# UoL-SignalProcessingGroup/SMC-NUTS

Hardware: AMD Instinct MI355X
Metric: leapfrog-steps/sec (higher is better)
Workload: dtype f64

## Files before the change

include/smcnuts_hip.h:

```cpp
#ifndef SMCNUTS_HIP_H
#define SMCNUTS_HIP_H

#include <stddef.h>
#include <stdint.h>

#ifdef __cplusplus
extern "C" {
#endif

typedef struct smcn_ctx smcn_ctx;

#define SMCN_MODEL_GAUSS 0
#define SMCN_MODEL_ARMA 1
#define SMCN_MODEL_PRMWCD 2
#define SMCN_MODEL_HOST 3
#define SMCN_MODEL_GLM 4
#define SMCN_MODEL_HGLM 5
#define SMCN_MODEL_CATEGORICAL 6
#define SMCN_MODEL_ORDINAL 7
#define SMCN_MODEL_MLGLM 8
#define SMCN_MODEL_WGLM 9
#define SMCN_MODEL_OGLM 10

#define SMCN_LKERNEL_FORWARD 0
// ... 46 lines not shown
int smcn_set_nuts_cap(smcn_ctx* ctx, int doublings, int widen);
int smcn_nuts_parked(smcn_ctx* ctx, int64_t* parked);
int smcn_set_nuts_requeue(smcn_ctx* ctx, int doublings);

int smcn_propose_nuts(smcn_ctx* ctx, double step_size, double phi, int max_depth, double delta_max,
                      int64_t iteration, const double* tape, const int64_t* tape_off);
int smcn_get_tree_stats(smcn_ctx* ctx, int32_t* nleap, int32_t* depth, int32_t* ndraws, int32_t* flags);
int smcn_last_leapfrogs(smcn_ctx* ctx, int64_t* total);
int smcn_get_density_parts(smcn_ctx* ctx, double* lpri0, double* llik0, double* lpri1, double* llik1);

int smcn_reweight(smcn_ctx* ctx, int lkernel);
int smcn_accept_reject(smcn_ctx* ctx, double phi, const double* u, int64_t iteration);
int smcn_reweight_asymptotic(smcn_ctx* ctx, double phi_old, double phi_new);
int smcn_set_logw_density_ratio(smcn_ctx* ctx, double phi_num, double phi_den);

int smcn_set_lkernel_values(smcn_ctx* ctx, const double* L, const double* q);

int smcn_gauss_lkernel_sums(smcn_ctx* ctx, const double* shift, double* sums);
int smcn_gauss_lkernel_logpdf(smcn_ctx* ctx, const double* mu_x, const double* m0, const double* B,
                              const double* U, double c0);
int smcn_gauss_lkernel_device(smcn_ctx* ctx, double info[4]);
int smcn_gauss_lkernel_buffers(smcn_ctx* ctx, int world, void** local_dev, void** gathered_dev);
int smcn_gauss_lkernel_stage(smcn_ctx* ctx, int stage, int world, double n_total, double info[4] );

int smcn_temper_partials(smcn_ctx* ctx, double phi_old, double phi_new, double out[4]);
int smcn_temper_bisect(smcn_ctx* ctx, double phi_old, double target, double* phi, int* status);
int smcn_temper_bisect_pass(smcn_ctx* ctx, int pass, double phi_old);
int smcn_temper_bisect_buffers(smcn_ctx* ctx, int world, void** local, void** gathered);
int smcn_temper_bisect_decide(smcn_ctx* ctx, int pass, int world, double target, double phi_old);
int smcn_temper_bisect_result(smcn_ctx* ctx, double* phi, int* status);

int smcn_eval_proposed_parts(smcn_ctx* ctx, int which);

int smcn_commit(smcn_ctx* ctx, int64_t* n_moved);

int smcn_fast_begin(smcn_ctx* ctx, int64_t K, int save_history, int world);
int smcn_fast_buffers(smcn_ctx* ctx, void** local_partials, void** gathered, int* nq);
int smcn_set_resample_uniforms(smcn_ctx* ctx, const double* u);
int smcn_step_begin(smcn_ctx* ctx, int64_t k);
int smcn_step_finish(smcn_ctx* ctx, int64_t k, int world, int rank, double n_total, double step_size,
                     double phi, int max_depth, double delta_max, int lkernel, int last,
                     const double* tape, const int64_t* tape_off);
int smcn_fast_read(smcn_ctx* ctx, double* hist, double* x_saved, double* logw_saved);
int smcn_fast_read_from(smcn_ctx* ctx, double* hist, double* x_saved, double* logw_saved, int64_t k_from);
int smcn_history_download(smcn_ctx* ctx, int64_t k_from, int64_t k_to, double* x_saved, double* logw_saved);
int smcn_fuse_begin(smcn_ctx* ctx, int Bmax, int world);
int smcn_fuse_buffers(smcn_ctx* ctx, void** local_partials, void** gathered, int* nq);
int smcn_fuse_run(smcn_ctx* ctx, int64_t k0, int B, int world, int rank, double n_total, double step_size,
                  double phi, int max_depth, double delta_max, int decided);
int smcn_fuse_decide(smcn_ctx* ctx, int64_t k0, int world, int rank, double n_total, double phi, int* resample);

typedef int (*smcn_host_target_fn)(void* user, int64_t n, int D, const double* x, int want_grad, double* lpri,
                                   double* llik, double* gpri, double* glik);
int smcn_set_host_target(smcn_ctx* ctx, smcn_host_target_fn fn, void* user);
int smcn_moment_sums_of(smcn_ctx* ctx, const double* v, int Dc, const double* shift, double* out);

int smcn_block_resample_local(smcn_ctx* ctx, int64_t k0);
int smcn_block_launch(smcn_ctx* ctx, int64_t k0, int B, double step_size, double phi, int max_depth,
                      double delta_max);
int smcn_block_post(smcn_ctx* ctx, int64_t k0, int B, int world);
int smcn_block_partials_get(smcn_ctx* ctx, int B, double* out);
int smcn_block_partials_set(smcn_ctx* ctx, int B, int world, const double* gathered);
int smcn_block_stats(smcn_ctx* ctx, int64_t k0, int B, int world, int rank, double n_total, double phi,
                     int final_block );
int smcn_block_wait(smcn_ctx* ctx, int B, int* n_ok, int* resample_next);
int smcn_block_commit(smcn_ctx* ctx, int64_t k0, int n_ok);
int smcn_block_ess(smcn_ctx* ctx, int B, double* out);
int smcn_fuse_finish(smcn_ctx* ctx, int64_t k0, int B, int world, int rank, double n_total, double phi,
                     int* n_ok);
#ifdef SMCN_LEGACY_ABI
int smcn_fuse_partials_get(smcn_ctx* ctx, int B, double* out);
int smcn_fuse_partials_set(smcn_ctx* ctx, int B, int world, const double* in);
#endif

int smcn_partials_get(smcn_ctx* ctx, double* out);
int smcn_partials_set_gathered(smcn_ctx* ctx, const double* in, int world);

int smcn_timers(smcn_ctx* ctx, double out[6], int reset);

int smcn_selftest_math(smcn_ctx* ctx, const double* x, int64_t n, double* out);
int smcn_measure_peaks(smcn_ctx* ctx, double out[3]);
int smcn_device_cache_trim(int device, int64_t* released_bytes, int64_t* idle_bytes);
int smcn_selftest_wide(smcn_ctx* ctx, int lanes, const double* x, int64_t n, double* out);

int smcn_comm_unique_id(char out[128]);
int smcn_comm_init(smcn_ctx* ctx, int rank, int world, const char id[128]);
int smcn_comm_destroy(smcn_ctx* ctx);
int smcn_comm_info(smcn_ctx* ctx, int out[3]);
int smcn_comm_allgather(smcn_ctx* ctx, const void* src_dev, void* dst_dev, int64_t n_doubles);
int smcn_comm_allgather_host(smcn_ctx* ctx, const double* src, int64_t n_doubles, double* dst );
int smcn_comm_alltoallv(smcn_ctx* ctx, const void* send_dev, const int64_t* send_counts, void* recv_dev,
                        const int64_t* recv_counts, int elem_doubles);
int smcn_buf_get(smcn_ctx* ctx, const void* dev, int64_t n_doubles, double* host);
int smcn_buf_set(smcn_ctx* ctx, void* dev, int64_t n_doubles, const double* host);
int smcn_buf_copy(smcn_ctx* ctx, void* dst_dev, const void* src_dev, int64_t n_doubles);

int smcn_gres_begin(smcn_ctx* ctx, int world, double* ttot_host );
int smcn_gres_buffers(smcn_ctx* ctx, void** ttot_local, void** ttot_all, void** keys_send, void** keys_recv,
                      void** rows_send, void** rows_recv);
int smcn_gres_plan(smcn_ctx* ctx, int world, int rank, const double* ttot_all_host ,
                   int64_t iteration, int32_t* dest_rank_host );
int smcn_gres_set_order(smcn_ctx* ctx, const int32_t* order );
int smcn_gres_reserve(smcn_ctx* ctx, int64_t n_requests_to_serve);
int smcn_gres_serve(smcn_ctx* ctx, int world, int rank, int64_t n_requests);
int smcn_gres_finish(smcn_ctx* ctx, int world, const double* loglik );

int smcn_bench_resample(smcn_ctx* ctx, int reps, int64_t iteration, double* ms_total);

int smcn_pointwise_dims(const smcn_ctx* ctx, int64_t* n_obs, int* n_cols);
int smcn_pointwise_loglik(smcn_ctx* ctx, const double* x , int64_t M, double* out );
int smcn_pointwise_partials(smcn_ctx* ctx, const double* x_or_null , const double* logw_or_null ,
                            int64_t M, double* out );
int smcn_pointwise_last_ms(const smcn_ctx* ctx, double* ms);

int smcn_psis_candidates(smcn_ctx* ctx, const double* x_or_null , const double* logw_or_null ,
                         int64_t M, double mw, int64_t S, double* cand );
int smcn_psis_body(smcn_ctx* ctx, const double* x_or_null , const double* logw_or_null , int64_t M,
                   double mw, int64_t S, const double* cutoff , double* body );
int smcn_psis_fit(smcn_ctx* ctx, const double* cand , const double* body ,
                  int64_t n_obs, double mw, int64_t S, double* out );
int smcn_psis_loo(smcn_ctx* ctx, const double* x_or_null , const double* logw_or_null , int64_t M,
                  double* out , double* head_or_null );
int smcn_psis_last_ms(const smcn_ctx* ctx, double* ms );

int smcn_predict_set_data(smcn_ctx* ctx, const double* block, int64_t len, int has_y);
int smcn_predict_dims(smcn_ctx* ctx, int64_t* n_rows, int* n_cols, int* has_y);
int smcn_predict_loglik(smcn_ctx* ctx, const double* x , int64_t M, double* out );
int smcn_predict_partials(smcn_ctx* ctx, const double* x_or_null , const double* logw_or_null ,
                          int64_t M, double* out );
int smcn_predict_last_ms(const smcn_ctx* ctx, double* ms);

int smcn_predict_draws(smcn_ctx* ctx, const double* x_or_null , const double* logw_or_null , int64_t M,
                       int64_t S, uint64_t seed, const int64_t* ancestors_or_null ,
                       const int64_t* new_group_or_null , int64_t s_first, int64_t s_count,
                       double* y_out , int64_t* ancestors_out , int64_t* n_bad_out);
int smcn_predict_draws_last_ms(const smcn_ctx* ctx, double* ms);

int smcn_summary_begin(smcn_ctx* ctx, const double* x_or_null , const double* logw_or_null ,
                       const double* v_or_null , int64_t M, int Dv, double* head_out );
int smcn_summary_weights(smcn_ctx* ctx, double lw_max, double lw_sum, double* mass_out);
int smcn_summary_select(smcn_ctx* ctx, int nq, const double* thresholds );
int smcn_summary_hist(smcn_ctx* ctx, int pass, int nq, double* out );
int smcn_summary_descend(smcn_ctx* ctx, int pass, int nq, const int32_t* digits ,
                         const double* residual );
int smcn_summary_values(smcn_ctx* ctx, int nq, double* out , double* nan_flags_out );
int smcn_summary_cdf(smcn_ctx* ctx, int T, const double* at , double* out );
int smcn_summary_last_ms(const smcn_ctx* ctx, double* ms);
int smcn_summary_pass_ms(const smcn_ctx* ctx, double* ms );

int smcn_cov_partials(smcn_ctx* ctx, double lw_max, const double* centre_or_null , int64_t slices,
                      double* out , double* centre_out );
int smcn_cov_dims(const smcn_ctx* ctx, int64_t* out );
int smcn_cov_last_ms(const smcn_ctx* ctx, double* ms);

int smcn_debug_profile(smcn_ctx* ctx, uint64_t out[16], int reset);

#ifdef __cplusplus
}
#endif
#endif
```

smcnuts_amd/_capi.py:

```python
import ctypes as C
import os

import numpy as np

from . import build as _build

MODEL_GAUSS, MODEL_ARMA, MODEL_PRMWCD, MODEL_HOST = 0, 1, 2, 3
MODEL_GLM = 4
MODEL_HGLM = 5
MODEL_CATEGORICAL = 6
MODEL_ORDINAL = 7
MODEL_MLGLM = 8
MODEL_WGLM = 9
MODEL_OGLM = 10
HOST_TARGET_FN = C.CFUNCTYPE(C.c_int, C.c_void_p, C.c_int64, C.c_int, C.POINTER(C.c_double), C.c_int,
                             C.POINTER(C.c_double), C.POINTER(C.c_double), C.POINTER(C.c_double),
                             C.POINTER(C.c_double))
LKERNEL_FORWARD, LKERNEL_GAUSSIAN = 0, 1

_dp = C.POINTER(C.c_double)
_ip = C.POINTER(C.c_int32)
_lp = C.POINTER(C.c_int64)
_ctx = C.c_void_p

# ... 4 lines not shown
    "smcn_ctx_destroy": ([_ctx], None),
    "smcn_dim": ([_ctx], C.c_int),
    "smcn_constrained_dim": ([_ctx], C.c_int),
    "smcn_fused_transitions": ([_ctx], C.c_int),
    "smcn_set_stream": ([_ctx, C.c_void_p], C.c_int),
    "smcn_synchronize": ([_ctx], C.c_int),
    "smcn_set_seed": ([_ctx, C.c_uint64], C.c_int),
    "smcn_set_state": ([_ctx, _dp, _dp], C.c_int),
    "smcn_get_state": ([_ctx, _dp, _dp, _dp], C.c_int),
    "smcn_get_proposal": ([_ctx, _dp, _dp, _dp, _dp], C.c_int),
    "smcn_set_momentum": ([_ctx, _dp], C.c_int),
    "smcn_set_proposal": ([_ctx, _dp, _dp, _dp], C.c_int),
    "smcn_target_eval": ([_ctx, _dp, C.c_int64, C.c_double, _dp, _dp, _dp, _dp], C.c_int),
    "smcn_target_constrain": ([_ctx, _dp, C.c_int64, _dp], C.c_int),
    "smcn_init_particles_std_normal": ([_ctx, C.c_double], C.c_int),
    "smcn_init_weights": ([_ctx, C.c_double, _dp], C.c_int),
    "smcn_normalise_partials": ([_ctx, _dp], C.c_int),
    "smcn_normalise_apply": ([_ctx, C.c_double], C.c_int),
    "smcn_normalise": ([_ctx, _dp, _dp], C.c_int),
    "smcn_moment_sums": ([_ctx, _dp, _dp], C.c_int),
    "smcn_resample_multinomial": ([_ctx, _dp, C.c_double, C.c_double, C.c_int64, _lp], C.c_int),
    "smcn_propose_nuts": ([_ctx, C.c_double, C.c_double, C.c_int, C.c_double, C.c_int64, _dp, _lp], C.c_int),
    "smcn_get_tree_stats": ([_ctx, _ip, _ip, _ip, _ip], C.c_int),
    "smcn_last_leapfrogs": ([_ctx, _lp], C.c_int),
    "smcn_get_density_parts": ([_ctx, _dp, _dp, _dp, _dp], C.c_int),
    "smcn_set_lkernel_values": ([_ctx, _dp, _dp], C.c_int),
    "smcn_reweight": ([_ctx, C.c_int], C.c_int),
    "smcn_accept_reject": ([_ctx, C.c_double, _dp, C.c_int64], C.c_int),
    "smcn_reweight_asymptotic": ([_ctx, C.c_double, C.c_double], C.c_int),
    "smcn_set_logw_density_ratio": ([_ctx, C.c_double, C.c_double], C.c_int),
    "smcn_gauss_lkernel_sums": ([_ctx, _dp, _dp], C.c_int),
    "smcn_gauss_lkernel_logpdf": ([_ctx, _dp, _dp, _dp, _dp, C.c_double], C.c_int),
    "smcn_gauss_lkernel_device": ([_ctx, _dp], C.c_int),
    "smcn_gauss_lkernel_buffers": ([_ctx, C.c_int, C.POINTER(C.c_void_p), C.POINTER(C.c_void_p)], C.c_int),
    "smcn_gauss_lkernel_stage": ([_ctx, C.c_int, C.c_int, C.c_double, _dp], C.c_int),
    "smcn_set_nuts_cap": ([_ctx, C.c_int, C.c_int], C.c_int),
    "smcn_set_nuts_requeue": ([_ctx, C.c_int], C.c_int),
    "smcn_nuts_parked": ([_ctx, C.POINTER(C.c_int64)], C.c_int),
    "smcn_temper_partials": ([_ctx, C.c_double, C.c_double, _dp], C.c_int),
    "smcn_temper_bisect": ([_ctx, C.c_double, C.c_double, C.POINTER(C.c_double), C.POINTER(C.c_int)], C.c_int),
    "smcn_temper_bisect_pass": ([_ctx, C.c_int, C.c_double], C.c_int),
    "smcn_temper_bisect_buffers": ([_ctx, C.c_int, C.POINTER(C.c_void_p), C.POINTER(C.c_void_p)], C.c_int),
    "smcn_temper_bisect_decide": ([_ctx, C.c_int, C.c_int, C.c_double, C.c_double], C.c_int),
    "smcn_temper_bisect_result": ([_ctx, C.POINTER(C.c_double), C.POINTER(C.c_int)], C.c_int),
    "smcn_eval_proposed_parts": ([_ctx, C.c_int], C.c_int),
    "smcn_commit": ([_ctx, _lp], C.c_int),
    "smcn_fast_begin": ([_ctx, C.c_int64, C.c_int, C.c_int], C.c_int),
    "smcn_fast_buffers": ([_ctx, C.POINTER(C.c_void_p), C.POINTER(C.c_void_p), C.POINTER(C.c_int)], C.c_int),
    "smcn_set_resample_uniforms": ([_ctx, _dp], C.c_int),
    "smcn_step_begin": ([_ctx, C.c_int64], C.c_int),
    "smcn_step_finish": ([_ctx, C.c_int64, C.c_int, C.c_int, C.c_double, C.c_double, C.c_double, C.c_int,
                          C.c_double, C.c_int, C.c_int, _dp, _lp], C.c_int),
    "smcn_fast_read": ([_ctx, _dp, _dp, _dp], C.c_int),
    "smcn_fast_read_from": ([_ctx, _dp, _dp, _dp, C.c_int64], C.c_int),
    "smcn_history_download": ([_ctx, C.c_int64, C.c_int64, _dp, _dp], C.c_int),
    "smcn_fuse_begin": ([_ctx, C.c_int, C.c_int], C.c_int),
    "smcn_fuse_buffers": ([_ctx, C.POINTER(C.c_void_p), C.POINTER(C.c_void_p), C.POINTER(C.c_int)], C.c_int),
    "smcn_fuse_run": ([_ctx, C.c_int64, C.c_int, C.c_int, C.c_int, C.c_double, C.c_double, C.c_double, C.c_int,
                       C.c_double, C.c_int], C.c_int),
    "smcn_set_resample_scheme": ([_ctx, C.c_int], C.c_int),
    "smcn_set_wide_eval": ([_ctx, C.c_int], C.c_int),
    "smcn_set_lane_grid": ([_ctx, C.c_int64], C.c_int),
    "smcn_set_lane_segments": ([_ctx, C.c_int], C.c_int),
    "smcn_set_host_target": ([_ctx, HOST_TARGET_FN, C.c_void_p], C.c_int),
    "smcn_moment_sums_of": ([_ctx, _dp, C.c_int, _dp, _dp], C.c_int),
    "smcn_block_resample_local": ([_ctx, C.c_int64], C.c_int),
    "smcn_block_launch": ([_ctx, C.c_int64, C.c_int, C.c_double, C.c_double, C.c_int, C.c_double], C.c_int),
    "smcn_block_post": ([_ctx, C.c_int64, C.c_int, C.c_int], C.c_int),
    "smcn_block_partials_get": ([_ctx, C.c_int, _dp], C.c_int),
    "smcn_block_partials_set": ([_ctx, C.c_int, C.c_int, _dp], C.c_int),
    "smcn_block_stats": ([_ctx, C.c_int64, C.c_int, C.c_int, C.c_int, C.c_double, C.c_double, C.c_int], C.c_int),
    "smcn_block_wait": ([_ctx, C.c_int, C.POINTER(C.c_int), C.POINTER(C.c_int)], C.c_int),
    "smcn_block_commit": ([_ctx, C.c_int64, C.c_int], C.c_int),
    "smcn_block_ess": ([_ctx, C.c_int, _dp], C.c_int),
    "smcn_fuse_decide": ([_ctx, C.c_int64, C.c_int, C.c_int, C.c_double, C.c_double, C.POINTER(C.c_int)], C.c_int),
    "smcn_fuse_finish": ([_ctx, C.c_int64, C.c_int, C.c_int, C.c_int, C.c_double, C.c_double,
                          C.POINTER(C.c_int)], C.c_int),
    "smcn_partials_get": ([_ctx, _dp], C.c_int),
    "smcn_partials_set_gathered": ([_ctx, _dp, C.c_int], C.c_int),
    "smcn_timers": ([_ctx, _dp, C.c_int], C.c_int),
    "smcn_selftest_math": ([_ctx, _dp, C.c_int64, _dp], C.c_int),
    "smcn_measure_peaks": ([_ctx, _dp], C.c_int),
    "smcn_selftest_wide": ([_ctx, C.c_int, _dp, C.c_int64, _dp], C.c_int),
    "smcn_device_cache_trim": ([C.c_int, C.POINTER(C.c_int64), C.POINTER(C.c_int64)], C.c_int),
    "smcn_debug_profile": ([_ctx, C.POINTER(C.c_uint64), C.c_int], C.c_int),
    "smcn_bench_resample": ([_ctx, C.c_int, C.c_int64, _dp], C.c_int),
    "smcn_comm_unique_id": ([C.c_char_p], C.c_int),
    "smcn_comm_init": ([_ctx, C.c_int, C.c_int, C.c_char_p], C.c_int),
    "smcn_comm_destroy": ([_ctx], C.c_int),
    "smcn_comm_info": ([_ctx, C.POINTER(C.c_int)], C.c_int),
    "smcn_comm_allgather": ([_ctx, C.c_void_p, C.c_void_p, C.c_int64], C.c_int),
    "smcn_comm_allgather_host": ([_ctx, _dp, C.c_int64, _dp], C.c_int),
    "smcn_comm_alltoallv": ([_ctx, C.c_void_p, _lp, C.c_void_p, _lp, C.c_int], C.c_int),
    "smcn_buf_get": ([_ctx, C.c_void_p, C.c_int64, _dp], C.c_int),
    "smcn_buf_set": ([_ctx, C.c_void_p, C.c_int64, _dp], C.c_int),
    "smcn_buf_copy": ([_ctx, C.c_void_p, C.c_void_p, C.c_int64], C.c_int),
    "smcn_gres_begin": ([_ctx, C.c_int, _dp], C.c_int),
    "smcn_gres_buffers": ([_ctx] + [C.POINTER(C.c_void_p)] * 6, C.c_int),
    "smcn_gres_plan": ([_ctx, C.c_int, C.c_int, _dp, C.c_int64, _ip], C.c_int),
    "smcn_gres_set_order": ([_ctx, _ip], C.c_int),
    "smcn_gres_reserve": ([_ctx, C.c_int64], C.c_int),
    "smcn_gres_serve": ([_ctx, C.c_int, C.c_int, C.c_int64], C.c_int),
    "smcn_gres_finish": ([_ctx, C.c_int, _dp], C.c_int),
    "smcn_pointwise_dims": ([_ctx, _lp, C.POINTER(C.c_int)], C.c_int),
    "smcn_pointwise_loglik": ([_ctx, _dp, C.c_int64, _dp], C.c_int),
    "smcn_pointwise_partials": ([_ctx, _dp, _dp, C.c_int64, _dp], C.c_int),
    "smcn_pointwise_last_ms": ([_ctx, _dp], C.c_int),
    "smcn_psis_candidates": ([_ctx, _dp, _dp, C.c_int64, C.c_double, C.c_int64, _dp], C.c_int),
    "smcn_psis_body": ([_ctx, _dp, _dp, C.c_int64, C.c_double, C.c_int64, _dp, _dp], C.c_int),
    "smcn_psis_fit": ([_ctx, _dp, _dp, C.c_int64, C.c_double, C.c_int64, _dp], C.c_int),
    "smcn_psis_loo": ([_ctx, _dp, _dp, C.c_int64, _dp, _dp], C.c_int),
    "smcn_psis_last_ms": ([_ctx, _dp], C.c_int),
    "smcn_predict_set_data": ([_ctx, _dp, C.c_int64, C.c_int], C.c_int),
    "smcn_predict_dims": ([_ctx, _lp, C.POINTER(C.c_int), C.POINTER(C.c_int)], C.c_int),
    "smcn_predict_loglik": ([_ctx, _dp, C.c_int64, _dp], C.c_int),
    "smcn_predict_partials": ([_ctx, _dp, _dp, C.c_int64, _dp], C.c_int),
    "smcn_predict_last_ms": ([_ctx, _dp], C.c_int),
    "smcn_predict_draws": ([_ctx, _dp, _dp, C.c_int64, C.c_int64, C.c_uint64, _lp, _lp, C.c_int64, C.c_int64, _dp, _lp,
                            _lp], C.c_int),
    "smcn_predict_draws_last_ms": ([_ctx, _dp], C.c_int),
    "smcn_summary_begin": ([_ctx, _dp, _dp, _dp, C.c_int64, C.c_int, _dp], C.c_int),
    "smcn_summary_weights": ([_ctx, C.c_double, C.c_double, _dp], C.c_int),
    "smcn_summary_select": ([_ctx, C.c_int, _dp], C.c_int),
    "smcn_summary_hist": ([_ctx, C.c_int, C.c_int, _dp], C.c_int),
    "smcn_summary_descend": ([_ctx, C.c_int, C.c_int, _ip, _dp], C.c_int),
    "smcn_summary_values": ([_ctx, C.c_int, _dp, _dp], C.c_int),
    "smcn_summary_cdf": ([_ctx, C.c_int, _dp, _dp], C.c_int),
    "smcn_summary_last_ms": ([_ctx, _dp], C.c_int),
    "smcn_summary_pass_ms": ([_ctx, _dp], C.c_int),
    "smcn_cov_partials": ([_ctx, C.c_double, _dp, C.c_int64, _dp, _dp], C.c_int),
    "smcn_cov_dims": ([_ctx, C.POINTER(C.c_int64)], C.c_int),
    "smcn_cov_last_ms": ([_ctx, _dp], C.c_int),
}

_lib = None


class SmcnError(RuntimeError):
    pass


def lib():
    global _lib
    if _lib is None:
        path = os.environ.get("SMCN_LIB") or _build.LIB
        if not os.path.exists(path):
            raise SmcnError(
                f"{path} is missing: build the HIP extension first "
                "(python -c 'import __graft_entry__ as g; g.build()').  There is no CPU fallback.")
        _lib = C.CDLL(path)
        for name, (args, res) in SIGNATURES.items():
            fn = getattr(_lib, name)
            fn.argtypes, fn.restype = args, res
    return _lib


def dptr(a):
    if a is None:
        return None
    assert a.dtype == np.float64 and a.flags["C_CONTIGUOUS"]
    return a.ctypes.data_as(_dp)


def iptr(a):
    return None if a is None else a.ctypes.data_as(_ip)

# ... 412 lines not shown
```

smcnuts_amd/csrc/smcn_api.hip:

```cpp
#include <hip/hip_runtime.h>

#include <dlfcn.h>

#include <cmath>
#include <cstdio>
#include <cstring>
#include <chrono>
#include <cstdlib>
#include <map>
#include <mutex>
#include <string>
#include <thread>
#include <unordered_map>
#include <vector>

#include "../../include/smcnuts_hip.h"
#include "smcn_nuts.hpp"
#include "smcn_nuts_wave.hpp"
#include "smcn_nuts_fin.hpp"
#include "smcn_nuts2.hpp"
#include "smcn_nuts3.hpp"
#include "smcn_temper.hpp"
#include "smcn_nuts_host.hpp"
#include "smcn_weights.hpp"
// ... 2762 lines not shown
    for (int64_t i = 0; i < n; ++i) dest_host[i] = tile[(size_t)i] / nt;
    (void)rank;
    return 0;
}
int smcn_gres_set_order(smcn_ctx* c, const int32_t* order) {
    CHECK_CTX(c);
    if (!order || c->g_world < 1) FAIL(c, "smcn_gres_set_order: bad arguments");
    const int64_t n = c->N;
    HIPC(c, hipMemcpyAsync(c->g_order, order, sizeof(int32_t) * n, hipMemcpyHostToDevice, c->stream));
    gres_permute_kernel<<<grid_for(n, 256), 256, 0, c->stream>>>(c->g_keys, c->g_order, n, c->g_keys_send);
    HIPC(c, hipGetLastError());
    HIPC(c, stream_wait(c->stream));
    return 0;
}
int smcn_gres_serve(smcn_ctx* c, int world, int rank, int64_t m) {
    CHECK_CTX(c);
    if (c->g_world != world || m < 0 || m > c->g_serve_cap) FAIL(c, "smcn_gres_serve: reserve first");
    const int64_t n = c->N;
    const int nt = grid_for(n, kScanTile);
    if (m > 0)
        gres_serve_kernel<<<grid_for(m, 256), 256, 0, c->stream>>>(c->g_keys_recv, m, c->g_toff_all, nt * world, rank * nt, nt,
                                                                   c->scan_local, n, c->x, c->D, c->g_rows_send);
    HIPC(c, hipGetLastError());
    return 0;
}
int smcn_gres_finish(smcn_ctx* c, int world, const double* loglik) {
    CHECK_CTX(c);
    if (c->g_world != world) FAIL(c, "smcn_gres_finish: call smcn_gres_begin first");
    if (!loglik && c->fast_K < 0) FAIL(c, "smcn_gres_finish: loglik needed outside the device-resident loop");
    const int64_t n = c->N;
    double ll = 0.0;
    if (loglik) {
        ll = *loglik;
    } else {
        HIPC(c, hipMemcpyAsync(&ll, c->ss + SS_LL, sizeof(double), hipMemcpyDeviceToHost, c->stream));
        HIPC(c, stream_wait(c->stream));
    }
    gres_scatter_kernel<<<grid_for(n, 256), 256, 0, c->stream>>>(c->g_rows_recv, c->g_order, n, c->D, c->x_tmp, c->logw,
                                                                 ll - log((double)(n * world)));
    HIPC(c, hipGetLastError());
    std::swap(c->x, c->x_tmp);
    return 0;
}

int smcn_selftest_math(smcn_ctx* c, const double* x, int64_t n, double* out) {
    CHECK_CTX(c);
    if (!x || !out || n < 1) FAIL(c, "smcn_selftest_math: bad arguments");
    int rc = ensure_stage(c, n);
    if (rc) return rc;
    if ((rc = ensure_stage2(c, 11 * n))) return rc;
    HIPC(c, hipMemcpyAsync(c->stage, x, sizeof(double) * n, hipMemcpyHostToDevice, c->stream));
    selftest_math_kernel<<<grid_for(n, 256), 256, 0, c->stream>>>(c->stage, n, c->stage2);
    HIPC(c, hipGetLastError());
    HIPC(c, hipMemcpyAsync(out, c->stage2, sizeof(double) * 11 * n, hipMemcpyDeviceToHost, c->stream));
    HIPC(c, stream_wait(c->stream));
    return 0;
}

int smcn_selftest_wide(smcn_ctx* c, int lanes, const double* x, int64_t n, double* out) {
    CHECK_CTX(c);
    if (c->model != SMCN_MODEL_ARMA || !c->lane_kernel) FAIL(c, "smcn_selftest_wide: arma contexts only");
    if (!x || !out || n < 1 || (lanes != 64 && lanes != 32 && lanes != 16 && lanes != 8 && lanes != 4)) FAIL(c, "smcn_selftest_wide: bad arguments");
    if (lanes >= 32 && c->arma_T < ArmaLaneModel::WIDE_MIN_T_ROWS) FAIL(c, "smcn_selftest_wide: 32 / 64 lanes per series take at least 130 observations");
    if (c->arma_T < ArmaLaneModel::WIDE_MIN_T || c->arma_T > ArmaLaneModel::YMAX)
        FAIL(c, "smcn_selftest_wide: the wide evaluation takes series of 64..384 observations");
    int rc = ensure_stage(c, 4 * n);
    if (rc) return rc;
    if ((rc = ensure_stage2(c, 8 * n))) return rc;
    HIPC(c, hipMemcpyAsync(c->stage, x, sizeof(double) * 4 * n, hipMemcpyHostToDevice, c->stream));
    const size_t lds = 8 * (ArmaLaneModel::YMAX + ArmaLaneModel::YPAD) + 16 * ArmaLaneModel::xch_pairs<4>();
    const int G = 64 / lanes;
    const int blocks = (int)((n + G - 1) / G);
    if (lanes == 64) selftest_wide_kernel<ArmaLaneModel, 64><<<blocks, 64, lds, c->stream>>>(c->mdata, c->stage, n, c->stage2);
    else if (lanes == 32) selftest_wide_kernel<ArmaLaneModel, 32><<<blocks, 64, lds, c->stream>>>(c->mdata, c->stage, n, c->stage2);
    else if (lanes == 16) selftest_wide_kernel<ArmaLaneModel, 16><<<blocks, 64, lds, c->stream>>>(c->mdata, c->stage, n, c->stage2);
    else if (lanes == 8) selftest_wide_kernel<ArmaLaneModel, 8><<<blocks, 64, lds, c->stream>>>(c->mdata, c->stage, n, c->stage2);
    else selftest_wide_kernel<ArmaLaneModel, 4><<<blocks, 64, lds, c->stream>>>(c->mdata, c->stage, n, c->stage2);
    HIPC(c, hipGetLastError());
    HIPC(c, hipMemcpyAsync(out, c->stage2, sizeof(double) * 8 * n, hipMemcpyDeviceToHost, c->stream));
    HIPC(c, stream_wait(c->stream));
    return 0;
}

}

static const char* kPwScope =
    "pointwise criteria cover the SMCN_MODEL_GLM families (bernoulli_logit, poisson_log, normal, neg_binomial_2_log) "
    "only; hierarchical, categorical, ordinal, arma, PRMwCD, Gaussian and host-evaluated targets are not implemented";

static const char* kPwWeighted =
    "pointwise criteria and LOO of a fit with weights (SMCN_MODEL_OGLM, flags & 2) are not implemented: what a weighted "
    "row's leave-one-out term and the standard error of the sum should be is not settled here";
static std::string pw_refusal(const smcn_ctx* c) {
    if (c->model == SMCN_MODEL_OGLM) return (c->reg.flags & 2) ? kPwWeighted : "";
    return c->model == SMCN_MODEL_GLM ? "" : kPwScope;
}
static PwArgs pw_args(const RegLayout& L, const double* md, const double* x, int64_t rs, int64_t cs, int64_t M, int64_t cps) {
    PwArgs a;
    a.md = md;
    a.x = x;
    a.rs = rs;
    a.cs = cs;
    a.M = M;
    a.cps = cps;
    a.fam = L.fam;
    a.n = (int)L.n;
    a.p = (int)L.p;
    a.Dc = L.Dc;
    return a;
}
static int pw_ensure(smcn_ctx* c, int64_t n) { return grow_scratch(c, c->pw_buf, c->pw_len, n); }
template <class F>
static void row_cap(int Dc, F&& f) {
    const int DP = (Dc + 1) & ~1;
    if (DP <= 16) f(std::integral_constant<int, 16>{});
    else if (DP <= 32) f(std::integral_constant<int, 32>{});
    else f(std::integral_constant<int, 64>{});
}
template <class F>
static void row_cap_disp(int Dc, int fam, F&& f) {
    row_cap(Dc, [&](auto dp) { fam >= 2 ? f(dp, std::true_type{}) : f(dp, std::false_type{}); });
}
template <class F>
static void row_cap_glm(const RegLayout& L, F&& f) {
    row_cap_disp(L.Dc, L.fam, [&](auto dp, auto disp) {
        L.model == SMCN_MODEL_OGLM ? f(dp, disp, std::true_type{}) : f(dp, disp, std::false_type{});
    });
}
template <class F>
static void cat_cap(int Dc, F&& f) {
    using std::integral_constant;
    if (Dc <= 4) f(integral_constant<int, 4>{}, integral_constant<int, 15>{});
    else if (Dc <= 8) f(integral_constant<int, 8>{}, integral_constant<int, 12>{});
    else if (Dc <= 16) f(integral_constant<int, 16>{}, integral_constant<int, 7>{});
    else if (Dc <= 32) f(integral_constant<int, 32>{}, integral_constant<int, 3>{});
    else f(integral_constant<int, 64>{}, integral_constant<int, 1>{});
}
struct Particles {
    const double* xd;
    int64_t rs, cs;
    double* lw;
};
static int stage_particles(smcn_ctx* c, const double* x, const double* logw, int64_t M, double* lw_stage, Particles* P) {
    if (!x) {
        *P = {c->x, 1, c->N, c->logw};
        return 0;
    }
    const int rc = ensure_stage(c, M * c->D);
    if (rc) return rc;
    HIPC(c, hipMemcpyAsync(c->stage, x, sizeof(double) * M * c->D, hipMemcpyHostToDevice, c->stream));
    if (logw) HIPC(c, hipMemcpyAsync(lw_stage, logw, sizeof(double) * M, hipMemcpyHostToDevice, c->stream));
    else HIPC(c, hipMemsetAsync(lw_stage, 0, sizeof(double) * M, c->stream));
    *P = {c->stage, c->D, 1, lw_stage};
    return 0;
}

extern "C" {

int smcn_pointwise_dims(const smcn_ctx* cc, int64_t* n_obs, int* n_cols) {
    smcn_ctx* c = const_cast<smcn_ctx*>(cc);
    if (!c) return -1;
    if (!pw_refusal(c).empty()) FAIL(c, "smcn_pointwise_dims: " + pw_refusal(c));
    if (n_obs) *n_obs = c->reg.n;
    if (n_cols) *n_cols = kPwCols;
    return 0;
}
// ... 1031 lines not shown
```

smcnuts_amd/csrc/smcn_nuts3.hpp:

```cpp
#pragma once
#include "smcn_nuts2.hpp"
#include <type_traits>

namespace smcn {

constexpr int kN3Block = 64;
constexpr int kN3ReadyWords = 64;


__constant__ double kArmaFinishTab[24] = {
    1.4426950408889634074, 6.93147180369123816490e-01, 1.90821492927058770002e-10,
    2.08767569878680989792e-09, 2.50521083854417187751e-08, 2.75573192239858906526e-07,
    2.75573192239858906526e-06, 2.48015873015873015873e-05, 1.98412698412698412698e-04,
    1.38888888888888888889e-03, 8.33333333333333333333e-03, 4.16666666666666666667e-02,
    1.66666666666666666667e-01,
    0.70710678118654752440,
    9.52380952380952380952e-02, 1.05263157894736842105e-01, 1.17647058823529411765e-01,
    1.33333333333333333333e-01, 1.53846153846153846154e-01, 1.81818181818181818182e-01,
    2.22222222222222222222e-01, 2.85714285714285714286e-01, 4.0e-01, 6.66666666666666666667e-01};

struct ArmaLaneModel {
    static constexpr int D = 4;
    static constexpr bool HAS_WIDE = true;
    using cptr = const __attribute__((address_space(4))) double*;
    int T;
    cptr y;

    __device__ __forceinline__ void init(const double* md) {
        T = __builtin_amdgcn_readfirstlane((int)((cptr)md)[0]);
        y = (cptr)md + 1;
    }

    __device__ __forceinline__ void eval(const double (&x)[4], double& lpri, double& llik, double (&gp)[4],
                                         double (&gl)[4]) const {
        double ss, gm, gb, gt;
        recur(x, ss, gm, gb, gt);
        finish(x, ss, gm, gb, gt, lpri, llik, gp, gl);
    }

    __device__ __forceinline__ void recur(const double (&x)[4], double& ss_o, double& gm_o, double& gb_o,
                                          double& gt_o) const {
        const double mu = x[0], beta = x[1], theta = x[2];
        const double nth = -theta, nbeta = -beta;
        double c0 = y[0];
        double err = fma(nbeta, mu, c0 - mu);
        double dm = -(1.0 + beta), db = -mu, dt = 0.0;
        double ss = err * err, gm = err * dm, gb = err * db, gt = 0.0;
        auto step = [&](double yp, double yt) {
            dt = fma(nth, dt, -err);
            dm = fma(nth, dm, -1.0);
            db = fma(nth, db, -yp);
            const double c = fma(nbeta, yp, yt - mu);
            err = fma(nth, err, c);
            ss = fma(err, err, ss);
            gm = fma(err, dm, gm);
            gb = fma(err, db, gb);
            gt = fma(err, dt, gt);
        };
        auto chunk = [&](double cy, const double (&Y)[8]) {
            step(cy, Y[0]);
#pragma unroll
            for (int k = 1; k < 8; ++k) step(Y[k - 1], Y[k]);
        };
        double A[8], B[8];
#pragma unroll
        for (int k = 0; k < 8; ++k) A[k] = y[1 + k];
        int t = 1;
        __builtin_amdgcn_s_waitcnt(0xC07F);
        auto round16 = [&](int tt) __attribute__((always_inline)) {
            step(c0, A[0]);
            __builtin_amdgcn_sched_barrier(0);
#pragma unroll
            for (int k = 0; k < 8; ++k) B[k] = y[tt + 8 + k];
            __builtin_amdgcn_sched_barrier(0);
#pragma unroll
            for (int k = 1; k < 8; ++k) step(A[k - 1], A[k]);
            c0 = A[7];
            __builtin_amdgcn_sched_barrier(0);
            step(c0, B[0]);
            __builtin_amdgcn_sched_barrier(0);
#pragma unroll
            for (int k = 0; k < 8; ++k) A[k] = y[tt + 16 + k];
            __builtin_amdgcn_sched_barrier(0);
#pragma unroll
            for (int k = 1; k < 8; ++k) step(B[k - 1], B[k]);
            c0 = B[7];
            __builtin_amdgcn_sched_barrier(0);
        };
        for (; t + 64 <= T; t += 64) {
            round16(t);
            round16(t + 16);
            round16(t + 32);
            round16(t + 48);
        }
        if (t + 32 <= T) {
            round16(t);
            round16(t + 16);
            t += 32;
        }
        if (t + 16 <= T) {
            round16(t);
            t += 16;
        }
        int rem = T - t;
        if (rem >= 8) {
#pragma unroll
            for (int k = 0; k < 8; ++k) B[k] = y[t + 8 + k];
            __builtin_amdgcn_sched_barrier(0);
            chunk(c0, A);
            c0 = A[7];
#pragma unroll
            for (int k = 0; k < 8; ++k) A[k] = B[k];
            rem -= 8;
        }
        if (rem >= 4) {
            step(c0, A[0]); step(A[0], A[1]); step(A[1], A[2]); step(A[2], A[3]);
            c0 = A[3];
#pragma unroll
            for (int k = 0; k < 4; ++k) A[k] = A[k + 4];
            rem -= 4;
        }
        if (rem >= 2) {
            step(c0, A[0]); step(A[0], A[1]);
            c0 = A[1];
            A[0] = A[2];
            rem -= 2;
        }
        if (rem >= 1) step(c0, A[0]);
        ss_o = ss; gm_o = gm; gb_o = gb; gt_o = gt;
    }

    __device__ __forceinline__ void finish(const double (&x)[4], double ss, double gm, double gb, double gt, double& lpri,
                                           double& llik, double (&gp)[4], double (&gl)[4]) const {
        const double mu = x[0], beta = x[1], theta = x[2], s = x[3];
        cptr tab = (cptr)kArmaFinishTab;
        asm volatile("" : "+s"(tab));
        double K[24];
#pragma unroll
        for (int i = 0; i < 24; ++i) K[i] = tab[i];
        double e2s;
        {
            const double t = 2.0 * s;
            const double k = __builtin_rint(t * K[0]);
            double r = fma(-k, K[1], t);
            r = fma(-k, K[2], r);
            double p = K[3];
#pragma unroll
            for (int i = 4; i <= 12; ++i) p = fma(p, r, K[i]);
            p = fma(p, r, 0.5);
            p = fma(p, r, 1.0);
            p = fma(p, r, 1.0);
            e2s = ldexp(p, (int)k);
        }
        const double w = rcp_nr(e2s);
        const double z2 = e2s * 0.16;
        double inv1pz, l1p;
        {
            const double u = 1.0 + z2;
            inv1pz = rcp_nr(u);
            int e = __builtin_amdgcn_frexp_exp(u);
            double m = __builtin_amdgcn_frexp_mant(u);
            const bool lo = m < K[13];
            m = lo ? m + m : m;
            e = lo ? e - 1 : e;
            const double f = (m - 1.0) * rcp_nr(m + 1.0);
            const double f2 = f * f;
            double p = K[14];
#pragma unroll
            for (int i = 15; i <= 23; ++i) p = fma(p, f2, K[i]);
            const double logm = fma(f * f2, p, f + f);
            const double ed = (double)e;
            const double lg = fma(ed, K[1], fma(ed, K[2], logm));
            l1p = fma(z2 - (u - 1.0), inv1pz, lg);
        }
        lpri = (-0.5 * kLog2Pi - 2.302585092994045684 - 0.005 * mu * mu)
             + (-0.5 * kLog2Pi - 0.6931471805599453094 - 0.125 * beta * beta)
             + (-0.5 * kLog2Pi - 0.6931471805599453094 - 0.125 * theta * theta)
             + (-kLogPi - 0.9162907318741550651 - l1p)
             + s;
        gp[0] = -0.01 * mu;
        gp[1] = -0.25 * beta;
        gp[2] = -0.25 * theta;
        gp[3] = 1.0 - 2.0 * (z2 * inv1pz);
        const double Td = (double)T;
        llik = -0.5 * Td * kLog2Pi - Td * s - 0.5 * ss * w;
        const double nw = -w;
        gl[0] = nw * gm;
        gl[1] = nw * gb;
        gl[2] = nw * gt;
        gl[3] = ss * w - Td;
    }


    static constexpr int YMAX = 384;
    static constexpr int WIDE_MIN_T = 64;
    static constexpr int WIDE_MIN_T_ROWS = 130;
    static constexpr int YPAD = 8;
    template <int A>
    static constexpr int xch_pairs() { return 2 * (64 / A); }
    template <int CTRL, int ROWS>
    static __device__ __forceinline__ double dpp_fill(double v, double fill) {
        int lo = __double2loint(v), hi = __double2hiint(v);
        lo = __builtin_amdgcn_update_dpp(__double2loint(fill), lo, CTRL, ROWS, 0xF, false);
        hi = __builtin_amdgcn_update_dpp(__double2hiint(fill), hi, CTRL, ROWS, 0xF, false);
        return __hiloint2double(hi, lo);
    }
    template <int A, int K>
    static __device__ __forceinline__ double seg_shift(double v, double fill) {
        static_assert(A == 64 || A == 32 || A == 16 || A == 8 || A == 4, "group widths: rows, a DPP row, half a row or a quad");
        if constexpr (A >= 32) return dpp_fill<0x110 + K, 0xF>(v, fill);
        else if constexpr (A >= 8) return dpp_mov<0x110 + K>(v);
        else return dpp_mov<(K == 1) ? 0x90 : 0x44>(v);
// ... 89 lines not shown
            e = first ? e_init : ei;
            dm = first ? dm_init : mi;
            db = first ? db_init : bi;
            dt = first ? 0.0 : ti;
        }
        double ss = first ? e * e : 0.0, gm = first ? e * dm : 0.0, gb = first ? e * db : 0.0, gt = 0.0;
        auto full_step = [&](double yp, double yt) __attribute__((always_inline)) {
            dt = fma(nth, dt, -e);
            dm = fma(nth, dm, -1.0);
            db = fma(nth, db, -yp);
            e = fma(nth, e, fma(nbeta, yp, yt - mu));
            ss = fma(e, e, ss);
            gm = fma(e, dm, gm);
            gb = fma(e, db, gb);
            gt = fma(e, dt, gt);
        };
        seg_walk(Yl + (i0 - 1), S, extra, full_step);
        if constexpr (A == 64) wave_sum4(ss, gm, gb, gt, ss, gm, gb, gt);
        else { ss = group_sum<A>(ss); gm = group_sum<A>(gm); gb = group_sum<A>(gb); gt = group_sum<A>(gt); }
        if (first) {
            d2 t;
            t.x = ss; t.y = gm;
            XCH[2 * g] = t;
            t.x = gb; t.y = gt;
            XCH[2 * g + 1] = t;
        }
        wave_exchange_fence();
        if (act) {
            const d2 r0 = XCH[2 * rank], r1 = XCH[2 * rank + 1];
            ss_o = r0.x; gm_o = r0.y; gb_o = r1.x; gt_o = r1.y;
        }
    }
};

template <class Model>
__global__ void __launch_bounds__(256) lane_eval_kernel(const double* mdata, const double* x, int64_t M, int64_t rs,
                                                        int64_t cs, double phi, double* logp, double* grad, int64_t grs,
                                                        int64_t gcs, double* lpri_o, double* llik_o) {
    constexpr int D = Model::D;
    Model model;
    model.init(mdata);
    for (int64_t i = (int64_t)blockIdx.x * blockDim.x + threadIdx.x; i < M; i += (int64_t)gridDim.x * blockDim.x) {
        double xv[D], lpri, llik, gp[D], gl[D];
#pragma unroll
        for (int k = 0; k < D; ++k) xv[k] = x[i * rs + k * cs];
        model.eval(xv, lpri, llik, gp, gl);
        const double lp0 = lpri + phi * llik;
        const bool bad = !finite_d(lp0);
        if (logp) logp[i] = bad ? -kInf : lp0;
        if (lpri_o) lpri_o[i] = lpri;
        if (llik_o) llik_o[i] = llik;
        if (grad) {
#pragma unroll
            for (int k = 0; k < D; ++k) grad[i * grs + k * gcs] = bad ? -kInf : fma(phi, gl[k], gp[k]);
        }
    }
}

template <class Model, int A>
__global__ void __launch_bounds__(64) selftest_wide_kernel(const double* mdata, const double* x, int64_t M, double* out) {
    using d2 = double __attribute__((ext_vector_type(2)));
    extern __shared__ d2 lds_sw[];
    Model model;
    model.init(mdata);
    double* const Yl = reinterpret_cast<double*>(lds_sw);
    d2* const XCH = reinterpret_cast<d2*>(Yl + Model::YMAX + Model::YPAD);
    const int lane = (int)threadIdx.x;
    for (int i = lane; i < model.T + Model::YPAD && i < Model::YMAX + Model::YPAD; i += 64) Yl[i] = i < model.T ? mdata[1 + i] : 0.0;
    wave_exchange_fence();
    constexpr int G = 64 / A;
    const int j = lane / A;
    const bool owner = (lane % A) == ((5 * j + 3) % A);
    const int64_t row = (int64_t)blockIdx.x * G + (G - 1 - j);
    const bool act = owner && row < M;
    double xv[4] = {0.0, 0.0, 0.0, 0.0};
    if (act)
        for (int c = 0; c < 4; ++c) xv[c] = x[row * 4 + c];
    double n0 = 0, n1 = 0, n2 = 0, n3 = 0, w0 = 0, w1 = 0, w2 = 0, w3 = 0;
    if (act) model.recur(xv, n0, n1, n2, n3);
    model.template recur_wide<A>(xv, act, __ballot(act), Yl, XCH, lane, w0, w1, w2, w3);
    if (act) {
        double* o = out + row * 8;
        o[0] = n0; o[1] = n1; o[2] = n2; o[3] = n3; o[4] = w0; o[5] = w1; o[6] = w2; o[7] = w3;
    }
}

__host__ __device__ constexpr int n3_lds_pairs(int D, int LC, int LF) {
    const int VH = n2_vp(D) / 2;
    return 4 + 2 + (VH + 1) + LC * (2 * VH + 1) + LF * 2 * VH;
}
__host__ __device__ constexpr int n3_ovf_pairs(int D, int LC, int LF) {
    const int VH = n2_vp(D) / 2;
    return (8 - LC) * (2 * VH + 1) + (8 - LF) * 2 * VH;
}

template <class Model>
__host__ __device__ constexpr int n3_lds_bytes(int LC, int LF) {
    int b = 16 * kN3Block * n3_lds_pairs(Model::D, LC, LF);
    if constexpr (Model::HAS_WIDE) b += 8 * (Model::YMAX + Model::YPAD) + 16 * Model::template xch_pairs<4>();
    return b;
}

__device__ __forceinline__ bool compact_mode(const Nuts2Args& a) { return a.logw0 != nullptr; }

template <class Model, bool TAPE, int LC, int LF, bool QUEUE = false, int WPE = 1>
__global__ void __launch_bounds__(kN3Block) __attribute__((amdgpu_waves_per_eu(WPE, WPE))) nuts3_kernel(Nuts2Args a) {
    constexpr int D = Model::D, VP = n2_vp(D), VH = VP / 2;
    constexpr int INSZ = n2_in_doubles(D), OUTSZ = n2_out_doubles(D);
    constexpr int RING = 0;
    constexpr int NST = RING + 4;
    constexpr int PREF = NST + 2;
    constexpr int CAND0 = PREF + VH + 1, CREC = 2 * VH + 1;
    constexpr int FIRST0 = CAND0 + LC * CREC, FREC = 2 * VH;
    constexpr int OCAND0 = 0, OFIRST0 = (8 - LC) * CREC, OVFP = n3_ovf_pairs(D, LC, LF);
    static_assert(FIRST0 + LF * FREC == n3_lds_pairs(D, LC, LF), "LDS layout");
    static_assert(LC >= 0 && LC <= 8 && LF >= 0 && LF <= 8, "levels");
    enum { INIT = 1, LEAF = 2, DONE = 3 };

    using d2 = double __attribute__((ext_vector_type(2)));
    using gptr2 = __attribute__((address_space(1))) d2*;
    using gcptr2 = const __attribute__((address_space(1))) d2*;
    using gcptr = const __attribute__((address_space(1))) double*;
    extern __shared__ d2 lds3[];
    const int lane = (int)threadIdx.x;
    d2* const L = lds3 + lane;
    gptr2 const O = (gptr2)a.ovf + ((int64_t)blockIdx.x * OVFP) * 64 + lane;

    Model model;
    model.init(a.mdata);
    double* const Yl = reinterpret_cast<double*>(lds3 + n3_lds_pairs(D, LC, LF) * 64);
    d2* const XCH = reinterpret_cast<d2*>(Yl + (Model::HAS_WIDE ? Model::YMAX + Model::YPAD : 0));
    bool wide_ok = false, wide_rows = false;
    if constexpr (Model::HAS_WIDE) {
        wide_ok = (a.wide & 1) != 0 && model.T >= Model::WIDE_MIN_T && model.T <= Model::YMAX;
        wide_rows = wide_ok && model.T >= Model::WIDE_MIN_T_ROWS;
        if (wide_ok) {
            for (int i = lane; i < model.T + Model::YPAD; i += kN3Block) Yl[i] = i < model.T ? ((gcptr)a.mdata)[1 + i] : 0.0;
            wave_exchange_fence();
        }
    }
    const int64_t N = a.N;
    const double eps = a.eps, phi = a.phi;
    const unsigned int w_quot = (unsigned int)N / gridDim.x, w_rem = (unsigned int)N % gridDim.x;
    const unsigned int w_count = QUEUE ? w_quot + (blockIdx.x < w_rem ? 1u : 0u) : (unsigned int)kN3Block;
    const int64_t w_start = QUEUE ? (int64_t)blockIdx.x * w_quot + (blockIdx.x < w_rem ? blockIdx.x : w_rem)
                                  : (int64_t)blockIdx.x * kN3Block;
    const int64_t p_first = w_start + lane;
    const bool live = QUEUE ? (unsigned int)lane < w_count : p_first < N;
    std::conditional_t<QUEUE, int64_t, const int64_t> p = p_first;
    const int64_t pc = live ? p_first : N - 1;
    bool have_next = false, own_wait = false;
    unsigned int i_next = 0u;
    int seg_next = 0;
    unsigned int n_ready = 0u;
    double lw_next = 0.0;
    double hx_next[D];
    int64_t toff_next = 0, tlen_next = 0;
    const int Bs = (QUEUE && a.seg_len > 0) ? a.seg_len : a.B;
    const int n_main = (a.B + Bs - 1) / Bs, b_tail = (QUEUE && a.seg_tail > 0) ? a.B - a.seg_tail : a.B;
    const unsigned int nseg = (unsigned int)(n_main + (b_tail < a.B ? 1 : 0));
    auto seg_begin = [&](int sg) __attribute__((always_inline)) {
        return sg < n_main ? sg * Bs : (sg == n_main ? b_tail : a.B);
    };
    int seg = 0, b_end = seg_begin(1);
    const unsigned int w_words = (w_quot + (w_rem ? 1u : 0u) + 63u) / 64u;
    unsigned long long rm = 0ull;
// ... 619 lines not shown
```

Before: 7.572 billion.

## Skip converged dm recurrence in ARMA gradient loop once wave-wide fixed point reached

After: 7.774 billion, median of 6. +2.7%, better.

```diff
diff --git a/include/smcnuts_hip.h b/include/smcnuts_hip.h
--- a/include/smcnuts_hip.h
+++ b/include/smcnuts_hip.h
@@ -152,6 +152,7 @@
 int smcn_measure_peaks(smcn_ctx* ctx, double out[3]);
 int smcn_device_cache_trim(int device, int64_t* released_bytes, int64_t* idle_bytes);
 int smcn_selftest_wide(smcn_ctx* ctx, int lanes, const double* x, int64_t n, double* out);
+int smcn_selftest_recur(smcn_ctx* ctx, const double* x, int64_t n, double* out);
 
 int smcn_comm_unique_id(char out[128]);
 int smcn_comm_init(smcn_ctx* ctx, int rank, int world, const char id[128]);
diff --git a/smcnuts_amd/_capi.py b/smcnuts_amd/_capi.py
--- a/smcnuts_amd/_capi.py
+++ b/smcnuts_amd/_capi.py
@@ -110,6 +110,7 @@
     "smcn_selftest_math": ([_ctx, _dp, C.c_int64, _dp], C.c_int),
     "smcn_measure_peaks": ([_ctx, _dp], C.c_int),
     "smcn_selftest_wide": ([_ctx, C.c_int, _dp, C.c_int64, _dp], C.c_int),
+    "smcn_selftest_recur": ([_ctx, _dp, C.c_int64, _dp], C.c_int),
     "smcn_device_cache_trim": ([C.c_int, C.POINTER(C.c_int64), C.POINTER(C.c_int64)], C.c_int),
     "smcn_debug_profile": ([_ctx, C.POINTER(C.c_uint64), C.c_int], C.c_int),
     "smcn_bench_resample": ([_ctx, C.c_int, C.c_int64, _dp], C.c_int),
diff --git a/smcnuts_amd/csrc/smcn_api.hip b/smcnuts_amd/csrc/smcn_api.hip
--- a/smcnuts_amd/csrc/smcn_api.hip
+++ b/smcnuts_amd/csrc/smcn_api.hip
@@ -2868,6 +2868,22 @@
     return 0;
 }
 
+int smcn_selftest_recur(smcn_ctx* c, const double* x, int64_t n, double* out) {
+    CHECK_CTX(c);
+    if (c->model != SMCN_MODEL_ARMA || !c->lane_kernel) FAIL(c, "smcn_selftest_recur: arma contexts only");
+    if (!x || !out || n < 1) FAIL(c, "smcn_selftest_recur: bad arguments");
+    int rc = ensure_stage(c, 4 * n);
+    if (rc) return rc;
+    if ((rc = ensure_stage2(c, 9 * n))) return rc;
+    HIPC(c, hipMemcpyAsync(c->stage, x, sizeof(double) * 4 * n, hipMemcpyHostToDevice, c->stream));
+    const int blocks = (int)((n + 63) / 64);
+    selftest_recur_kernel<ArmaLaneModel><<<blocks, 64, 0, c->stream>>>(c->mdata, c->stage, n, c->stage2);
+    HIPC(c, hipGetLastError());
+    HIPC(c, hipMemcpyAsync(out, c->stage2, sizeof(double) * 9 * n, hipMemcpyDeviceToHost, c->stream));
+    HIPC(c, stream_wait(c->stream));
+    return 0;
+}
+
 }
 
 static const char* kPwScope =
diff --git a/smcnuts_amd/csrc/smcn_nuts3.hpp b/smcnuts_amd/csrc/smcn_nuts3.hpp
--- a/smcnuts_amd/csrc/smcn_nuts3.hpp
+++ b/smcnuts_amd/csrc/smcn_nuts3.hpp
@@ -38,96 +38,137 @@
         finish(x, ss, gm, gb, gt, lpri, llik, gp, gl);
     }
 
+    template <bool SETTLE = true>
     __device__ __forceinline__ void recur(const double (&x)[4], double& ss_o, double& gm_o, double& gb_o,
                                           double& gt_o) const {
+        int sw;
+        recur_sw<SETTLE>(x, ss_o, gm_o, gb_o, gt_o, sw);
+    }
+
+    template <bool SETTLE>
+    __device__ __forceinline__ void recur_sw(const double (&x)[4], double& ss_o, double& gm_o, double& gb_o, double& gt_o,
+                                             int& sw_o) const {
+        using full_t = std::false_type;
+        using settled_t = std::true_type;
         const double mu = x[0], beta = x[1], theta = x[2];
         const double nth = -theta, nbeta = -beta;
         double c0 = y[0];
         double err = fma(nbeta, mu, c0 - mu);
         double dm = -(1.0 + beta), db = -mu, dt = 0.0;
+        double d1 = 0.0;
         double ss = err * err, gm = err * dm, gb = err * db, gt = 0.0;
-        auto step = [&](double yp, double yt) {
+        auto step = [&](auto S, int k, double yp, double yt) __attribute__((always_inline)) {
             dt = fma(nth, dt, -err);
-            dm = fma(nth, dm, -1.0);
+            if constexpr (!decltype(S)::value) dm = fma(nth, dm, -1.0);
             db = fma(nth, db, -yp);
             const double c = fma(nbeta, yp, yt - mu);
             err = fma(nth, err, c);
             ss = fma(err, err, ss);
-            gm = fma(err, dm, gm);
+            gm = fma(err, (decltype(S)::value && !(k & 1)) ? d1 : dm, gm);
             gb = fma(err, db, gb);
             gt = fma(err, dt, gt);
         };
-        auto chunk = [&](double cy, const double (&Y)[8]) {
-            step(cy, Y[0]);
-#pragma unroll
-            for (int k = 1; k < 8; ++k) step(Y[k - 1], Y[k]);
+        auto chunk = [&](double cy, const double (&Y)[8]) __attribute__((always_inline)) {
+            step(full_t{}, 0, cy, Y[0]);
+#pragma unroll
+            for (int k = 1; k < 8; ++k) step(full_t{}, k, Y[k - 1], Y[k]);
         };
         double A[8], B[8];
 #pragma unroll
         for (int k = 0; k < 8; ++k) A[k] = y[1 + k];
         int t = 1;
         __builtin_amdgcn_s_waitcnt(0xC07F);
-        auto round16 = [&](int tt) __attribute__((always_inline)) {
-            step(c0, A[0]);
+        auto round16 = [&](auto S, int tt) __attribute__((always_inline)) {
+            step(S, 0, c0, A[0]);
             __builtin_amdgcn_sched_barrier(0);
 #pragma unroll
             for (int k = 0; k < 8; ++k) B[k] = y[tt + 8 + k];
             __builtin_amdgcn_sched_barrier(0);
 #pragma unroll
-            for (int k = 1; k < 8; ++k) step(A[k - 1], A[k]);
+            for (int k = 1; k < 8; ++k) step(S, k, A[k - 1], A[k]);
             c0 = A[7];
             __builtin_amdgcn_sched_barrier(0);
-            step(c0, B[0]);
+            step(S, 0, c0, B[0]);
             __builtin_amdgcn_sched_barrier(0);
 #pragma unroll
             for (int k = 0; k < 8; ++k) A[k] = y[tt + 16 + k];
             __builtin_amdgcn_sched_barrier(0);
 #pragma unroll
-            for (int k = 1; k < 8; ++k) step(B[k - 1], B[k]);
+            for (int k = 1; k < 8; ++k) step(S, k, B[k - 1], B[k]);
             c0 = B[7];
             __builtin_amdgcn_sched_barrier(0);
         };
-        for (; t + 64 <= T; t += 64) {
-            round16(t);
-            round16(t + 16);
-            round16(t + 32);
-            round16(t + 48);
-        }
-        if (t + 32 <= T) {
-            round16(t);
-            round16(t + 16);
-            t += 32;
-        }
-        if (t + 16 <= T) {
-            round16(t);
-            t += 16;
-        }
-        int rem = T - t;
-        if (rem >= 8) {
-#pragma unroll
-            for (int k = 0; k < 8; ++k) B[k] = y[t + 8 + k];
-            __builtin_amdgcn_sched_barrier(0);
-            chunk(c0, A);
-            c0 = A[7];
-#pragma unroll
-            for (int k = 0; k < 8; ++k) A[k] = B[k];
-            rem -= 8;
-        }
-        if (rem >= 4) {
-            step(c0, A[0]); step(A[0], A[1]); step(A[1], A[2]); step(A[2], A[3]);
-            c0 = A[3];
-#pragma unroll
-            for (int k = 0; k < 4; ++k) A[k] = A[k + 4];
-            rem -= 4;
-        }
-        if (rem >= 2) {
-            step(c0, A[0]); step(A[0], A[1]);
-            c0 = A[1];
-            A[0] = A[2];
-            rem -= 2;
-        }
-        if (rem >= 1) step(c0, A[0]);
-        ss_o = ss; gm_o = gm; gb_o = gb; gt_o = gt;
+        auto rest = [&](auto LONG) __attribute__((always_inline)) {
+            constexpr full_t S{};
+            if constexpr (decltype(LONG)::value) {
+                for (; t + 64 <= T; t += 64) {
+                    round16(S, t);
+                    round16(S, t + 16);
+                    round16(S, t + 32);
+                    round16(S, t + 48);
+                }
+                if (t + 32 <= T) {
+                    round16(S, t);
+                    round16(S, t + 16);
+                    t += 32;
+                }
+            }
+            if (t + 16 <= T) {
+                round16(S, t);
+                t += 16;
+            }
+            int rem = T - t;
+            if (rem >= 8) {
+#pragma unroll
+                for (int k = 0; k < 8; ++k) B[k] = y[t + 8 + k];
+                __builtin_amdgcn_sched_barrier(0);
+                chunk(c0, A);
+                c0 = A[7];
+#pragma unroll
+                for (int k = 0; k < 8; ++k) A[k] = B[k];
+                rem -= 8;
+            }
+            if (rem >= 4) {
+                step(S, 0, c0, A[0]); step(S, 1, A[0], A[1]); step(S, 0, A[1], A[2]); step(S, 1, A[2], A[3]);
+                c0 = A[3];
+#pragma unroll
+                for (int k = 0; k < 4; ++k) A[k] = A[k + 4];
+                rem -= 4;
+            }
+            if (rem >= 2) {
+                step(S, 0, c0, A[0]); step(S, 1, A[0], A[1]);
+                c0 = A[1];
+                A[0] = A[2];
+                rem -= 2;
+            }
+            if (rem >= 1) step(S, 0, c0, A[0]);
+        };
+        int sw = 0;
+        if constexpr (!SETTLE) {
+            rest(std::true_type{});
+        } else {
+            bool settled = false;
+            while (t + 32 <= T) {
+                round16(full_t{}, t);
+                round16(full_t{}, t + 16);
+                t += 32;
+                d1 = fma(nth, dm, -1.0);
+                const double d2 = fma(nth, d1, -1.0);
+                if (__ballot(!(d2 == dm)) == 0) {
+                    settled = true;
+                    break;
+                }
+            }
+            if (settled) {
+                sw = t - 1;
+                for (; t + 32 <= T; t += 32) {
+                    round16(settled_t{}, t);
+                    round16(settled_t{}, t + 16);
+                }
+            }
+            rest(std::false_type{});
+        }
+        ss_o = ss; gm_o = gm; gb_o = gb; gt_o = gt; sw_o = sw;
     }
 
     __device__ __forceinline__ void finish(const double (&x)[4], double ss, double gm, double gb, double gt, double& lpri,
@@ -383,6 +424,24 @@
     if (act) {
         double* o = out + row * 8;
         o[0] = n0; o[1] = n1; o[2] = n2; o[3] = n3; o[4] = w0; o[5] = w1; o[6] = w2; o[7] = w3;
+    }
+}
+
+template <class Model>
+__global__ void __launch_bounds__(64) selftest_recur_kernel(const double* mdata, const double* x, int64_t M, double* out) {
+    Model model;
+    model.init(mdata);
+    const int64_t row = (int64_t)blockIdx.x * 64 + threadIdx.x;
+    if (row < M) {
+        double xv[4];
+#pragma unroll
+        for (int c = 0; c < 4; ++c) xv[c] = x[row * 4 + c];
+        double f0, f1, f2, f3, s0, s1, s2, s3;
+        int sw;
+        model.template recur<false>(xv, f0, f1, f2, f3);
+        model.template recur_sw<true>(xv, s0, s1, s2, s3, sw);
+        double* o = out + row * 9;
+        o[0] = f0; o[1] = f1; o[2] = f2; o[3] = f3; o[4] = s0; o[5] = s1; o[6] = s2; o[7] = s3; o[8] = (double)sw;
     }
 }
 
```
